# flock-lab/flock

Hardware: AMD Instinct MI355X
Metric: NEXMark rows/sec per node (q3 join, q5 agg) (higher is better)
Workload: dtype int32; 1 GPU; NEXMark q5 hopping(10,5) over 1087 s x 1000000 events/s per GPU; query=q5, input_rows_per_gpu=1000040000, windows_per_gpu=216, parallelism=one GPU, one process

## Files before the change

### flock_amd/csrc/q5.hip

```cpp
#include <algorithm>

#include "sort.hpp"

using namespace flockgpu;

namespace {

constexpr int kQ5Iters = 8;
constexpr int kQ5Tile = kBlock * 4 * kQ5Iters;
constexpr int kHist = 4096;
constexpr int kHistPad = 64;
constexpr int kSlots = kHist / 2;
constexpr int kSlotBits = 11;
static_assert(kSlots == (1 << kSlotBits), "slot bits");
constexpr int kLdsMaxProbe = 24;
constexpr uint32_t kFib = 0x9E3779B1u;
constexpr int kHotMin = 16;
constexpr int kMaxWinPanes = 8;
constexpr uint32_t kWideTile = 0x40000000u;

struct PaneDesc {
    int64_t base;
    uint64_t cnt_off;
    uint32_t range;
    uint32_t pad;
};

struct WinDesc {
    int64_t base;
    uint32_t range;
    int32_t pane_lo, pane_hi;
    uint32_t pad;
};

__device__ __forceinline__ int lds_hash_insert(uint64_t *tab, uint32_t key, uint32_t c) {
    uint32_t s = (key * kFib) >> (32 - kSlotBits);
    const uint64_t mine = ((uint64_t)key << 32) | c;
#pragma unroll 1
    for (int probe = 0; probe < kLdsMaxProbe; ++probe) {
        uint64_t cur = __hip_atomic_load(&tab[s], __ATOMIC_RELAXED, __HIP_MEMORY_SCOPE_WORKGROUP);
        if (cur == 0) {
            cur = atomicCAS(reinterpret_cast<unsigned long long *>(&tab[s]), 0ull, (unsigned long long)mine);
            if (cur == 0) return 2;
        }
        if ((uint32_t)(cur >> 32) == key) {
            atomicAdd(reinterpret_cast<unsigned long long *>(&tab[s]), (unsigned long long)c);
            return 1;
        }
        s = (s + 1) & (kSlots - 1);
    }
    return 0;
}

__device__ __forceinline__ void table_add(uint64_t *tab, uint32_t cap, uint32_t key, uint32_t c, uint32_t *used, uint32_t *err) {
    uint32_t s = (uint32_t)(((uint64_t)(key * kFib) * cap) >> 32);
    const uint64_t mine = ((uint64_t)key << 32) | c;
#pragma unroll 1
    for (uint32_t probe = 0, lim = cap < 2048u ? cap : 2048u; probe < lim; ++probe) {
        uint64_t cur = __hip_atomic_load(&tab[s], __ATOMIC_RELAXED, __HIP_MEMORY_SCOPE_AGENT);
        if (cur == 0) {
            uint64_t expected = 0;
            if (__hip_atomic_compare_exchange_strong(&tab[s], &expected, mine, __ATOMIC_RELAXED, __ATOMIC_RELAXED,
                                                     __HIP_MEMORY_SCOPE_AGENT)) {
                if (*used == 0) *used = 1u;
                return;
            }
            cur = expected;
        }
        if ((uint32_t)(cur >> 32) == key) {
            __hip_atomic_fetch_add(&tab[s], (uint64_t)c, __ATOMIC_RELAXED, __HIP_MEMORY_SCOPE_AGENT);
            return;
        }
        s = (s + 1 == cap) ? 0 : s + 1;
    }
    atomicOr(err, 1u);
}

__device__ __forceinline__ uint32_t table_find(const uint64_t *tab, uint32_t cap, uint32_t key) {
    uint32_t s = (uint32_t)(((uint64_t)(key * kFib) * cap) >> 32);
#pragma unroll 1
    for (uint32_t probe = 0, lim = cap < 2048u ? cap : 2048u; probe < lim; ++probe) {
        const uint64_t cur = tab[s];
        if (cur == 0) return 0;
        if ((uint32_t)(cur >> 32) == key) return (uint32_t)cur;
        s = (s + 1 == cap) ? 0 : s + 1;
    }
    return 0;
}

struct FlushArgs {
    PaneDesc pane;
    int32_t wp0, wp1;
    const int32_t *pane_win_idx;
    uint32_t *counters;
    uint64_t *tables;
    uint32_t cap;
    uint32_t *tab_used;
    uint32_t *err;
    bool c16 = false;
    unsigned long long *tab_rows = nullptr;
};

// ... 78 lines not shown
    uint64_t capacity, budget_bytes;
    PaneDesc *panes;
    WinDesc *wins;
    uint64_t *info;
};
__device__ __forceinline__ void q5_layout_block(const int32_t *__restrict__ rng, const int32_t *__restrict__ pane_win_ptr,
                                                const int64_t *__restrict__ seg_off, int32_t n_panes, int32_t n_win,
                                                uint64_t capacity, uint64_t budget_bytes, PaneDesc *__restrict__ panes,
                                                WinDesc *__restrict__ wins, uint64_t *__restrict__ info) {
    __shared__ uint64_t s_wave[kWavesPerBlock];
    __shared__ uint64_t s_carry;
    __shared__ int s_ok;
    const int lane = lane_id(), wave = threadIdx.x >> 6;
    if (threadIdx.x == 0) {
        s_carry = 0;
        s_ok = 1;
    }
    __syncthreads();
    for (int32_t p0 = 0; p0 < n_panes; p0 += kBlock) {
        const int32_t p = p0 + (int32_t)threadIdx.x;
        int64_t base = 0, range = 0;
        if (p < n_panes && pane_win_ptr[p + 1] != pane_win_ptr[p] && seg_off[2 * p + 1] > seg_off[2 * p]) {
            int32_t mn = 0x7fffffff, mx = (int32_t)0x80000000;
            for (int b = 0; b < kRangeBlocks; ++b) {
                mn = min(mn, rng[((size_t)p * kRangeBlocks + b) * 2]);
                mx = max(mx, rng[((size_t)p * kRangeBlocks + b) * 2 + 1]);
            }
            if (mn <= mx && !q5_pane_layout(mn, mx, &base, &range)) {
                s_ok = 0;
                range = 0;
            }
        }
        const uint64_t incl = wave_incl_scan_u64((uint64_t)range);
        if (lane == 63) s_wave[wave] = incl;
        __syncthreads();
        uint64_t off = s_carry + incl - (uint64_t)range;
        for (int v = 0; v < wave; ++v) off += s_wave[v];
        if (p < n_panes) panes[p] = PaneDesc{base, off, (uint32_t)range, 0};
        __syncthreads();
        if (threadIdx.x == kBlock - 1) s_carry = off + (uint64_t)range;
        __syncthreads();
    }
    const uint64_t cnt_total = s_carry;
    __syncthreads();
    uint64_t scan = 0;
    for (int32_t w = threadIdx.x; w < n_win; w += kBlock) {
        WinDesc d = wins[w];
        int64_t lo = INT64_MAX, hi = INT64_MIN;
        for (int32_t p = d.pane_lo; p < d.pane_hi; ++p) {
            const PaneDesc pd = panes[p];
            if (pd.range) {
                lo = lo < pd.base ? lo : pd.base;
                hi = hi > pd.base + (int64_t)pd.range ? hi : pd.base + (int64_t)pd.range;
            }
        }
        d.base = 0;
        d.range = 0;
        if (lo < hi) {
            if (hi - lo >= (int64_t(1) << 31)) s_ok = 0;
            else {
                d.base = lo;
                d.range = (uint32_t)(hi - lo);
                scan += (uint64_t)(hi - lo);
            }
        }
        wins[w] = d;
    }
    scan = wave_sum_u64(scan);
    if (lane == 0) s_wave[wave] = scan;
    __syncthreads();
    if (threadIdx.x == 0) {
        uint64_t scan_total = 0;
        for (int v = 0; v < kWavesPerBlock; ++v) scan_total += s_wave[v];
        const bool ok = s_ok && cnt_total <= capacity && cnt_total * 4 <= budget_bytes && scan_total * 4 <= 2 * budget_bytes;
        info[0] = cnt_total;
        info[1] = scan_total;
        info[2] = ok ? 1 : 0;
    }
}

__global__ __launch_bounds__(kBlock) void q5_clear_kernel(uint32_t *__restrict__ counters, uint64_t cnt_host,
                                                          uint64_t cnt_from, uint64_t *__restrict__ tables, uint64_t table_words,
                                                          uint64_t *__restrict__ meta, uint64_t meta_words, int32_t *__restrict__ slow_list,
                                                          uint32_t *__restrict__ block_max, uint64_t block_max_words, int c16, LayoutArgs lay) {
    if (lay.rng && blockIdx.x == 0) q5_layout_block(lay.rng, lay.pane_win_ptr, lay.seg_off, lay.n_panes, lay.n_win, lay.capacity, lay.budget_bytes, lay.panes, lay.wins, lay.info);
    uint64_t cnt = cnt_host;
    if (c16) cnt = (cnt + 1) / 2;
    const uint64_t i0 = (uint64_t)blockIdx.x * kBlock + threadIdx.x, stride = (uint64_t)gridDim.x * kBlock;
    const uint4 z = make_uint4(0, 0, 0, 0);
    for (uint64_t i = i0 + cnt_from / 4; i * 4 < cnt + 3; i += stride) {
        uint32_t *p = counters + i * 4;
        __builtin_nontemporal_store(0u, p);
        __builtin_nontemporal_store(0u, p + 1);
        __builtin_nontemporal_store(0u, p + 2);
        __builtin_nontemporal_store(0u, p + 3);
    }
    for (uint64_t i = i0; i * 2 < table_words; i += stride) {
        if (i * 2 + 1 < table_words) reinterpret_cast<uint4 *>(tables)[i] = z;
        else tables[i * 2] = 0;
    }
    for (uint64_t i = i0; i < meta_words; i += stride) meta[i] = 0;
    for (uint64_t i = i0; i < block_max_words; i += stride) block_max[i] = 0;
    if (i0 == 0) slow_list[0] = 0;
}

template <bool kWeighted>
__device__ __forceinline__ void q5_count_tile(const int32_t *__restrict__ auction, const uint32_t *__restrict__ weight, const SegTiles &st,
                                              const PaneDesc *__restrict__ panes, const int32_t *__restrict__ pane_win_ptr,
                                              const int32_t *__restrict__ pane_win_idx, uint32_t *counters, uint64_t *tables, uint32_t cap,
                                              uint32_t *tab_used, uint32_t *err, int32_t *slow_list, unsigned long long *pane_wsum, const int32_t tile,
                                              uint32_t *hist, int32_t *s_red, unsigned long long *s_w, const bool c16, unsigned long long *tab_rows) {
    const TileRange tr = locate_tile(st, tile, kQ5Tile);
    FlushArgs f;
    f.c16 = c16;
    f.tab_rows = tab_rows ? tab_rows + tr.seg : nullptr;
    f.wp0 = pane_win_ptr[tr.seg];
    f.wp1 = pane_win_ptr[tr.seg + 1];
    if (f.wp0 == f.wp1) return;
    f.pane = panes[tr.seg];
    f.pane_win_idx = pane_win_idx;
    f.counters = counters;
    f.tables = tables;
    f.cap = cap;
    f.tab_used = tab_used;
    f.err = err;
    const bool full_tile = tr.lo == tr.tile_begin && tr.hi == tr.tile_begin + kQ5Tile;
    if (kWeighted) {
        unsigned long long wsum = 0;
        constexpr int kChunks = kQ5Tile / kBlock, kBatch = 8;
#pragma unroll 1
        for (int c0 = 0; c0 < kChunks; c0 += kBatch) {
            int32_t kk[kBatch];
            uint32_t ww[kBatch];
#pragma unroll
            for (int b = 0; b < kBatch; ++b) {
                const int64_t r = tr.tile_begin + (int64_t)(c0 + b) * kBlock + threadIdx.x;
                const bool in = full_tile || (r >= tr.lo && r < tr.hi);
                kk[b] = in ? __builtin_nontemporal_load(&auction[r]) : 0;
                ww[b] = in ? __builtin_nontemporal_load(&weight[r]) : 0u;
            }
#pragma unroll
            for (int b = 0; b < kBatch; ++b)
                if (ww[b]) {
                    emit_pair(kk[b], ww[b], f);
                    wsum += ww[b];
                }
        }
        wsum = wave_sum_u64(wsum);
        if (lane_id() == 0) s_w[threadIdx.x >> 6] = wsum;
        __syncthreads();
        if (threadIdx.x == 0 && pane_wsum) {
            const unsigned long long tot = s_w[0] + s_w[1] + s_w[2] + s_w[3];
            if (tot) atomicAdd(&pane_wsum[tr.seg], tot);
        }
        return;
    }
    {
        uint4 *z = reinterpret_cast<uint4 *>(hist);
        for (int s = threadIdx.x; s < (kHist + kHistPad) / 4; s += kBlock) z[s] = make_uint4(0, 0, 0, 0);
    }
    const int lane = lane_id(), wave = threadIdx.x >> 6;
    int32_t k[kQ5Iters][4];
    const int32_t key0 = full_tile ? 0 : auction[tr.lo];
    if (full_tile) {
#pragma unroll
        for (int it = 0; it < kQ5Iters; ++it) {
            const int64_t r0 = tr.tile_begin + it * (kBlock * 4) + threadIdx.x * 4;
            const int4 t = stream_load4(auction + r0);
            k[it][0] = t.x; k[it][1] = t.y; k[it][2] = t.z; k[it][3] = t.w;
// ... 413 lines not shown
        if (lane_id() == 0) {
            s_best[threadIdx.x >> 6] = best;
            s_groups[threadIdx.x >> 6] = g;
        }
        __syncthreads();
        if (threadIdx.x == 0) {
            uint32_t b = 0;
            uint64_t gs = 0;
#pragma unroll
            for (int v = 0; v < kWavesPerBlock; ++v) {
                b = max(b, s_best[v]);
                gs += s_groups[v];
            }
            if (b) block_max[(size_t)w * gridDim.x + blockIdx.x] = b;
            if (b) atomicMax(reinterpret_cast<unsigned long long *>(&win_max[w]), (unsigned long long)b);
            if (gs) atomicAdd(reinterpret_cast<unsigned long long *>(&win_groups[w]), (unsigned long long)gs);
        }
    }
}

template <bool SELECT, bool k16>
__global__ __launch_bounds__(kBlock) void q5_hop2_scan_kernel(const PaneDesc *__restrict__ panes, const int32_t *__restrict__ pane_wa,
                                                              const int32_t *__restrict__ pane_wb, const uint32_t *__restrict__ counters,
                                                              const uint64_t *__restrict__ tables, uint32_t cap, const uint32_t *__restrict__ tab_used,
                                                              uint64_t *win_max, uint64_t *win_groups, uint32_t *block_max, uint32_t *cursor,
                                                              uint32_t out_cap, int32_t *out_win, int32_t *out_key, const uint64_t *__restrict__ spec_info,
                                                              unsigned long long *pane_sum) {
    constexpr int G = k16 ? 8 : 4;
    __shared__ uint32_t s_best[2][kWavesPerBlock];
    __shared__ uint64_t s_groups[3][kWavesPerBlock];
    if (spec_info && !spec_info[2]) return;
    const int32_t p = blockIdx.y;
    const int32_t wa = pane_wa[p], wb = pane_wb[p];
    if (wa < 0 && wb < 0) return;
    const PaneDesc pd = panes[p];
    const PaneDesc prev = wa >= 0 ? panes[p - 1] : PaneDesc{0, 0, 0, 0};
    const bool two_b = wb >= 0 && pane_wa[p + 1] == wb;
    const PaneDesc next = two_b ? panes[p + 1] : PaneDesc{0, 0, 0, 0};
    const uint32_t mx_a = SELECT && wa >= 0 ? (uint32_t)win_max[wa] : 0u, mx_b = SELECT && wb >= 0 ? (uint32_t)win_max[wb] : 0u;
    bool act_a = wa >= 0, act_b = wb >= 0;
    if (SELECT) {
        act_a = act_a && mx_a != 0 && block_max[((size_t)wa * 2 + 1) * gridDim.x + blockIdx.x] == mx_a;
        act_b = act_b && mx_b != 0 && block_max[((size_t)wb * 2 + 0) * gridDim.x + blockIdx.x] == mx_b;
        if (!act_a && !act_b) return;
    }
    const bool tab_a = wa >= 0 && tab_used[wa] != 0, tab_b = wb >= 0 && tab_used[wb] != 0;
    const uint64_t *ta = tables + (size_t)(wa >= 0 ? wa : 0) * cap, *tb = tables + (size_t)(wb >= 0 ? wb : 0) * cap;
    uint32_t best_a = 0, best_b = 0, groups_a = 0, groups_b = 0;
    uint64_t sum = 0;
    auto take = [&](uint32_t c, int32_t key, int32_t w, uint32_t mx, uint32_t &best, uint32_t &groups) {
        if (SELECT) {
            const bool hit = c == mx;
            const uint64_t b = __ballot(hit);
            if (b) {
                const int leader = __ffsll((unsigned long long)b) - 1;
                uint32_t base = 0;
                if (lane_id() == leader) base = atomicAdd(cursor, (uint32_t)__popcll((unsigned long long)b));
                base = __builtin_amdgcn_readlane(base, leader);
                const uint32_t pos = base + mbcnt(b);
                if (hit && pos < out_cap) {
                    out_win[pos] = w;
                    out_key[pos] = key;
                }
            }
        } else {
            best = max(best, c);
            groups += c != 0;
        }
    };
    auto unpack = [&](const uint4 v, uint32_t (&c)[G]) {
        if constexpr (k16) {
            const uint32_t w[4] = {v.x, v.y, v.z, v.w};
#pragma unroll
            for (int j = 0; j < 4; ++j) {
                c[2 * j] = w[j] & 0xFFFFu;
                c[2 * j + 1] = w[j] >> 16;
            }
        } else {
            c[0] = v.x; c[1] = v.y; c[2] = v.z; c[3] = v.w;
        }
    };
    const uint32_t ng = pd.range / G;
    const uint32_t *mine = counters + (k16 ? pd.cnt_off / 2 : pd.cnt_off), *theirs = counters + (k16 ? next.cnt_off / 2 : next.cnt_off);
    for (uint32_t i = blockIdx.x * kBlock + threadIdx.x; i < ng; i += gridDim.x * kBlock) {
        const int64_t k0 = pd.base + (int64_t)i * G;
        uint32_t me[G];
        unpack(*reinterpret_cast<const uint4 *>(mine + (uint64_t)i * 4), me);
        if (k16 && !SELECT) {
#pragma unroll
            for (int j = 0; j < G; ++j) sum += me[j];
        }
        if (act_b) {
            uint32_t c[G];
#pragma unroll
            for (int j = 0; j < G; ++j) c[j] = me[j];
            const uint64_t idx = (uint64_t)(k0 - next.base);
            if (idx < (uint64_t)next.range) {
                uint32_t o[G];
                unpack(*reinterpret_cast<const uint4 *>(theirs + (k16 ? idx / 2 : idx)), o);
#pragma unroll
                for (int j = 0; j < G; ++j) c[j] += o[j];
            }
            if (tab_b) {
#pragma unroll
                for (int j = 0; j < G; ++j) c[j] += table_find(tb, cap, (uint32_t)(int32_t)(k0 + j));
            }
#pragma unroll
            for (int j = 0; j < G; ++j) take(c[j], (int32_t)(k0 + j), wb, mx_b, best_b, groups_b);
        }
        if (act_a && !((uint64_t)(k0 - prev.base) < (uint64_t)prev.range)) {
            uint32_t c[G];
#pragma unroll
            for (int j = 0; j < G; ++j) c[j] = me[j];
            if (tab_a) {
#pragma unroll
                for (int j = 0; j < G; ++j) c[j] += table_find(ta, cap, (uint32_t)(int32_t)(k0 + j));
            }
#pragma unroll
            for (int j = 0; j < G; ++j) take(c[j], (int32_t)(k0 + j), wa, mx_a, best_a, groups_a);
        }
    }
    if (tab_b && act_b) {
        for (uint32_t sl = blockIdx.x * kBlock + threadIdx.x; sl < cap; sl += gridDim.x * kBlock) {
            const uint64_t e = tb[sl];
            if (!e) continue;
            const int64_t key = (int32_t)(uint32_t)(e >> 32);
            if ((uint64_t)(key - pd.base) < (uint64_t)pd.range || (uint64_t)(key - next.base) < (uint64_t)next.range) continue;
            if (SELECT) {
                if ((uint32_t)e == mx_b) {
                    const uint32_t pos = atomicAdd(cursor, 1u);
                    if (pos < out_cap) {
                        out_win[pos] = wb;
                        out_key[pos] = (int32_t)key;
                    }
                }
            } else {
                best_b = max(best_b, (uint32_t)e);
                groups_b += 1;
            }
        }
    }
    if (!SELECT) {
        const uint32_t ba = wave_max_u32(best_a), bb = wave_max_u32(best_b);
        const uint64_t ga = wave_sum_u64(groups_a), gb = wave_sum_u64(groups_b), gs = k16 ? wave_sum_u64(sum) : 0;
        if (lane_id() == 0) {
            s_best[0][threadIdx.x >> 6] = ba;
            s_best[1][threadIdx.x >> 6] = bb;
            s_groups[0][threadIdx.x >> 6] = ga;
            s_groups[1][threadIdx.x >> 6] = gb;
            s_groups[2][threadIdx.x >> 6] = gs;
        }
        __syncthreads();
        if (threadIdx.x < 2) {
            const int r = threadIdx.x;
            const int32_t w = r == 0 ? wa : wb;
            uint32_t b = 0;
            uint64_t g = 0;
#pragma unroll
            for (int v = 0; v < kWavesPerBlock; ++v) {
                b = max(b, s_best[r][v]);
                g += s_groups[r][v];
            }
            if (w >= 0) {
                if (b) block_max[((size_t)w * 2 + (r == 0 ? 1 : 0)) * gridDim.x + blockIdx.x] = b;
                if (b) atomicMax(reinterpret_cast<unsigned long long *>(&win_max[w]), (unsigned long long)b);
                if (g) atomicAdd(reinterpret_cast<unsigned long long *>(&win_groups[w]), (unsigned long long)g);
// ... 494 lines not shown
    if (preclean.size() != 2) preclean.assign(2, 0);
    LayoutArgs lay{};
    uint64_t clean_upto = 0;
    const bool c16 = !weight && !part && !wide_mode && hop2 && ctx->host_i64["q5.no_c16"].empty();
    auto words_of = [&](uint64_t n_counters) -> uint64_t { return c16 ? (n_counters + 1) / 2 : n_counters; };
    if (speculate) {
        FG_TRY(arena_get_t(ctx, "q5.counters", (size_t)words_of((uint64_t)hint[0] + (uint64_t)hint[0] / 8) + 8, &counters));
        capacity = (ctx->arena["q5.counters"].cap / sizeof(uint32_t) - 8) * (c16 ? 2 : 1);
        if (preclean[0] == (int64_t)reinterpret_cast<uintptr_t>(counters)) clean_upto = (uint64_t)preclean[1];
        {
            std::vector<int64_t> &wsig = ctx->host_i64["q5.wins_sig"];
            std::vector<int64_t> wnow;
            wnow.reserve((size_t)2 * n_win + 2);
            wnow.push_back((int64_t)reinterpret_cast<uintptr_t>(d_wins));
            for (int w = 0; w < n_win; ++w) {
                wnow.push_back(win->win_pane_lo[w]);
                wnow.push_back(win->win_pane_hi[w]);
            }
            if (wsig != wnow) {
                std::copy(wins.begin(), wins.end(), h_wins);
                FG_HIP(ctx, hipMemcpyAsync(d_wins, h_wins, wins.size() * sizeof(WinDesc), hipMemcpyHostToDevice, ctx->stream));
                wsig = wnow;
            }
        }
        lay = LayoutArgs{d_rng, d_ptr, st.seg_off, n_panes, n_win, capacity, budget, d_panes, d_wins, d_info};
        cnt_total = (uint64_t)hint[0];
        scan_total = (uint64_t)hint[1];
    } else {
        FG_TRY(upload_layout());
        FG_TRY(arena_get_t(ctx, "q5.counters", (size_t)words_of(cnt_total) + 8, &counters));
    }
    preclean[0] = preclean[1] = 0;

    const size_t n_meta = (size_t)2 * n_win + 1 + ((size_t)n_win + 1) / 2 + 1;
    const size_t n_meta_all = n_meta + (size_t)2 * std::max(n_panes, 0);
    uint64_t *d_meta = nullptr, *h_meta = nullptr;
    FG_TRY(arena_get_t(ctx, "q5.meta", n_meta_all, &d_meta));
    unsigned long long *d_pane_sum = reinterpret_cast<unsigned long long *>(d_meta + n_meta), *d_tab_rows = d_pane_sum + std::max(n_panes, 0);
    FG_TRY(pinned_get_t(ctx, "q5.meta", n_meta, &h_meta));
    uint32_t *d_cursor = reinterpret_cast<uint32_t *>(d_meta + 2 * n_win), *d_err = d_cursor + 1, *d_used = d_cursor + 2;

    unsigned long long *d_wsum = nullptr, *h_wsum = nullptr;
    if (weight && n_panes > 0) {
        FG_TRY(arena_get_t(ctx, "q5.pane_weight", (size_t)n_panes + 1, &d_wsum));
        FG_TRY(pinned_get_t(ctx, "q5.pane_weight", (size_t)n_panes + 1, &h_wsum));
    }
    double rpg = ctx->q5_rows_per_group < 1.0 ? 1.0 : ctx->q5_rows_per_group;
    uint64_t cap64 = dense ? 1024 : std::max<uint64_t>(1024, (uint64_t)((double)max_win_rows / rpg * 2.0) + 64);
    uint32_t out_cap = 1u << 16;
    std::vector<int32_t> h_win, h_key;
    uint32_t n_sel = 0;
    const int32_t *sel_win = nullptr, *sel_key = nullptr;
    bool fin_sorted = false;
    const int64_t *fin_off = nullptr;
    const int32_t *fin_auction = nullptr;
    const uint64_t *fin_num = nullptr;
    uint32_t h_slow_count = 0;
    for (int attempt = 0;; ++attempt) {
        if (attempt > 8 || cap64 >= (uint64_t(1) << 31))
            return fail(ctx, FLOCKGPU_ERR_CAPACITY, "q5: hash table capacity %llu still overflows", (unsigned long long)cap64);
        const uint32_t cap = (uint32_t)cap64;
        const uint64_t *spec_info = speculate ? d_info : nullptr;
        uint64_t *tables = nullptr;
        FG_TRY(arena_get_t(ctx, "q5.tables", (size_t)cap * std::max(n_win, 1), &tables));
        int32_t *o_win = nullptr, *o_key = nullptr, *slow_list = nullptr;
        FG_TRY(arena_get_t(ctx, "q5.sel_win", out_cap, &o_win));
        FG_TRY(arena_get_t(ctx, "q5.sel_key", out_cap, &o_key));
        FG_TRY(arena_get_t(ctx, "q5.slow_list", (size_t)st.n_tiles + 2, &slow_list));
        const uint64_t per_win = n_win > 0 ? std::max<uint64_t>(cap, scan_total / n_win / 4) : cap;
        const bool pane_walk = hop2;
        const uint64_t per_pane = n_panes > 0 ? std::max<uint64_t>(cap, cnt_total / (uint64_t)n_panes / 4) : cap;
        const int hop2_blocks = c16 ? 16 : 32;
        const unsigned gx = (unsigned)std::min<int64_t>(std::max<int64_t>(div_up((int64_t)(pane_walk ? per_pane : per_win), kBlock * 2), 1), pane_walk ? hop2_blocks : 64);
        uint32_t *block_max = nullptr;
        const uint64_t n_block_max = (uint64_t)gx * std::max(n_win, 1) * (pane_walk ? 2 : 1);
        FG_TRY(arena_get_t(ctx, "q5.block_max", (size_t)n_block_max, &block_max));
        {
            const uint64_t clear_words = std::max<uint64_t>({words_of(speculate ? capacity : cnt_total), (uint64_t)cap * n_win, (uint64_t)n_meta_all, n_block_max});
            const unsigned cg = (unsigned)std::max<int64_t>(1, std::min<int64_t>(div_up((int64_t)clear_words / 4 + 1, kBlock), (int64_t)ctx->num_cus * 16));
            {
                LaunchScope ls(ctx, "q5_clear_kernel");
                hipLaunchKernelGGL(q5_clear_kernel, dim3(cg), dim3(kBlock), 0, ctx->stream, counters, speculate ? capacity : cnt_total,
                                   (attempt == 0 && speculate) ? (clean_upto & ~uint64_t(3)) : uint64_t(0), tables, (uint64_t)cap * n_win, d_meta, (uint64_t)n_meta_all,
                                   slow_list, block_max, n_block_max, c16 ? 1 : 0, speculate ? lay : LayoutArgs{});
                if (speculate) clean_upto = std::max(clean_upto, words_of(capacity));
            }
            FG_TRY(check_launch(ctx, "q5_clear_kernel"));
        }
        if (d_wsum) FG_HIP(ctx, hipMemsetAsync(d_wsum, 0, sizeof(unsigned long long) * (size_t)n_panes, ctx->stream));
        uint32_t nd = 0;
        if (wide_mode && dense) {
            uint32_t max_range = 0;
            for (int p = 0; p < n_panes; ++p) max_range = std::max(max_range, panes[(size_t)p].range);
            nd = (uint32_t)div_up((int64_t)max_range, int64_t(1) << kPartShift) + 1;
        }
        const bool wide = wide_mode && dense && nd >= 2 && nd <= (uint32_t)kPartMaxDigits && st.n_tiles > 0 && n_win > 0;
        wide_ran = wide;
        uint32_t *d_sample = nullptr, *h_sample = nullptr;
        FG_TRY(arena_get_t(ctx, "q5.part_sample", 4, &d_sample));
        FG_TRY(pinned_get_t(ctx, "q5.part_sample", 4, &h_sample));
        h_sample[0] = h_sample[1] = 0;
        if (wide) {
            SegTiles st4;
            FG_TRY(build_seg_tiles(ctx, "q5.part", sb.data(), se.data(), n_panes, kPartTile, &st4));
            const int64_t slots = (int64_t)st4.n_tiles * (nd + 1);
            if (slots >= (int64_t(1) << 31)) return fail(ctx, FLOCKGPU_ERR_UNSUPPORTED, "q5: too many (pane, digit, tile) slots for the partition pass");
            int32_t *off_mat = nullptr, *part_keys = nullptr;
            uint16_t *part_low = nullptr;
            FG_TRY(arena_get_t(ctx, "q5.part_hist", (size_t)slots + 4, &off_mat));
            FG_TRY(arena_get_t(ctx, "q5.part_keys", (size_t)st4.n_tiles * kPartTile + 4, &part_keys));
            FG_TRY(arena_get_t(ctx, "q5.part_low", (size_t)st4.n_tiles * kPartTile + 8, &part_low));
            FG_HIP(ctx, hipMemsetAsync(d_sample, 0, 2 * sizeof(uint32_t), ctx->stream));
            {
                LaunchScope ls(ctx, "q5_part_tile_kernel");
                hipLaunchKernelGGL(q5_part_tile_kernel, dim3((unsigned)st4.n_tiles), dim3(kBlock), 0, ctx->stream, auction, st4, d_panes, d_ptr, nd, off_mat, part_keys,
                                   part_low, d_sample);
            }
            FG_TRY(check_launch(ctx, "q5_part_tile_kernel"));
            {
                LaunchScope ls(ctx, "q5_bucket_count_kernel");
                hipLaunchKernelGGL(q5_bucket_count_kernel, dim3(nd, (unsigned)n_panes), dim3(kBlock), 0, ctx->stream, part_keys, part_low, st4, d_panes, d_ptr, d_idx, nd,
                                   off_mat, counters, tables, cap, d_used, d_err);
            }
            FG_TRY(check_launch(ctx, "q5_bucket_count_kernel"));
            FG_HIP(ctx, hipMemcpyAsync(h_sample, d_sample, 2 * sizeof(uint32_t), hipMemcpyDeviceToHost, ctx->stream));
        } else if (st.n_tiles > 0 && n_win > 0) {
            {
                LaunchScope ls(ctx, "q5_count_kernel");
                hipLaunchKernelGGL(weight ? q5_count_kernel<true> : q5_count_kernel<false>, dim3((unsigned)st.n_tiles), dim3(kBlock), 0,
                                   ctx->stream, auction, weight, st, d_panes, d_ptr, d_idx, counters, tables, cap, d_used, d_err,
                                   slow_list, spec_info, d_wsum, c16 ? 1 : 0, c16 ? d_tab_rows : (unsigned long long *)nullptr);
            }
            FG_TRY(check_launch(ctx, "q5_count_kernel"));
            if (d_wsum) FG_HIP(ctx, hipMemcpyAsync(h_wsum, d_wsum, sizeof(unsigned long long) * (size_t)n_panes, hipMemcpyDeviceToHost, ctx->stream));
            {
                LaunchScope ls(ctx, "q5_count_slow_kernel");
                const unsigned gs = (unsigned)std::min<int64_t>(st.n_tiles, (int64_t)ctx->num_cus * 8);
                hipLaunchKernelGGL(weight ? q5_count_slow_kernel<true> : q5_count_slow_kernel<false>, dim3(gs), dim3(kBlock), 0,
                                   ctx->stream, auction, weight, st, d_panes, d_ptr, d_idx, counters, tables, cap, d_used, d_err,
                                   slow_list, spec_info, c16 ? 1 : 0, c16 ? d_tab_rows : (unsigned long long *)nullptr);
            }
            FG_TRY(check_launch(ctx, "q5_count_slow_kernel"));
        }
        if (part) {
            const int64_t tab0 = ((int64_t)cnt_total + 3) & ~int64_t(3);
            std::vector<int64_t> xb((size_t)2 * n_win), xe((size_t)2 * n_win);
            for (int w = 0; w < n_win; ++w) {
                xb[2 * w] = (int64_t)panes[w].cnt_off;
                xe[2 * w] = (int64_t)panes[w].cnt_off + (int64_t)panes[w].range;
                xb[2 * w + 1] = tab0 + (int64_t)w * cap;
                xe[2 * w + 1] = xb[2 * w + 1] + cap;
            }
            SegTiles sx;
            FG_TRY(build_seg_tiles(ctx, "q5.partial", xb.data(), xe.data(), 2 * n_win, kFlagTile, &sx));
            uint32_t *x_flags = nullptr, *x_counts = nullptr;
            uint64_t *x_base = nullptr;
            int64_t *d_xoff = nullptr, *h_xoff = nullptr;
            FG_TRY(arena_get_t(ctx, "q5.partial_flags", (size_t)sx.n_tiles * kBlock + 4, &x_flags));
            FG_TRY(arena_get_t(ctx, "q5.partial_counts", (size_t)sx.n_tiles * kWavesPerBlock + 4, &x_counts));
            FG_TRY(arena_get_t(ctx, "q5.partial_base", (size_t)sx.n_tiles + 1, &x_base));
            FG_TRY(arena_get_t(ctx, "q5.partial_off", (size_t)2 * n_win + 1, &d_xoff));
            FG_TRY(pinned_get_t(ctx, "q5.partial_off", (size_t)2 * n_win + 1, &h_xoff));
            if (sx.n_tiles > 0) {
                LaunchScope ls(ctx, "q5_partial_flag_kernel");
                hipLaunchKernelGGL(q5_partial_flag_kernel, dim3((unsigned)sx.n_tiles), dim3(kBlock), 0, ctx->stream, sx, counters, tables,
                                   tab0, x_flags, x_counts);
            }
            FG_TRY(check_launch(ctx, "q5_partial_flag_kernel"));
            FG_TRY(launch_tile_scan(ctx, x_counts, sx.n_tiles, x_base, sx.tile_first, sx.n_seg, d_xoff));
            FG_HIP(ctx, hipMemcpyAsync(h_xoff, d_xoff, sizeof(int64_t) * ((size_t)2 * n_win + 1), hipMemcpyDeviceToHost, ctx->stream));
            FG_HIP(ctx, hipMemcpyAsync(h_meta, d_meta, sizeof(uint64_t) * n_meta, hipMemcpyDeviceToHost, ctx->stream));
            FG_HIP(ctx, hipStreamSynchronize(ctx->stream));
            if (reinterpret_cast<const uint32_t *>(h_meta + 2 * n_win)[1]) {
                cap64 *= 4;
                continue;
            }
            const int64_t n_out = h_xoff[2 * n_win];
            if (n_out >= (int64_t(1) << 31)) return fail(ctx, FLOCKGPU_ERR_UNSUPPORTED, "q5 partial: more than 2^31 groups");
            int32_t *p_key = nullptr;
            uint32_t *p_cnt = nullptr;
            FG_TRY(arena_get_t(ctx, "q5.partial_key", (size_t)n_out + 4, &p_key));
            FG_TRY(arena_get_t(ctx, "q5.partial_cnt", (size_t)n_out + 4, &p_cnt));
            if (sx.n_tiles > 0 && n_out > 0) {
                LaunchScope ls(ctx, "q5_partial_emit_kernel");
                hipLaunchKernelGGL(q5_partial_emit_kernel, dim3((unsigned)sx.n_tiles), dim3(kBlock), 0, ctx->stream, sx, x_flags, x_counts,
                                   x_base, counters, tables, tab0, d_panes, p_key, p_cnt);
            }
            FG_TRY(check_launch(ctx, "q5_partial_emit_kernel"));
            std::vector<int64_t> &poffs = ctx->host_i64["q5.partial_pane_offsets"];
            poffs.resize((size_t)n_win + 1);
            for (int w = 0; w <= n_win; ++w) poffs[w] = h_xoff[2 * w];
            part->auction = p_key;
            part->count = p_cnt;
            part->pane_out_offsets = poffs.data();
            part->rows = n_out;
            return FLOCKGPU_OK;
        }
        if (n_win > 0 && pane_walk) {
            {
                LaunchScope ls(ctx, "q5_max_kernel");
                hipLaunchKernelGGL((c16 ? q5_hop2_scan_kernel<false, true> : q5_hop2_scan_kernel<false, false>), dim3(gx, (unsigned)n_panes), dim3(kBlock), 0, ctx->stream, d_panes, d_roles,
                                   d_roles + role_a.size(), counters, tables, cap, d_used, d_meta, d_meta + n_win, block_max, d_cursor, out_cap, o_win, o_key, spec_info, d_pane_sum);
            }
            FG_TRY(check_launch(ctx, "q5_max_kernel"));
            {
                LaunchScope ls(ctx, "q5_select_kernel");
                hipLaunchKernelGGL((c16 ? q5_hop2_scan_kernel<true, true> : q5_hop2_scan_kernel<true, false>), dim3(gx, (unsigned)n_panes), dim3(kBlock), 0, ctx->stream, d_panes, d_roles,
                                   d_roles + role_a.size(), counters, tables, cap, d_used, d_meta, d_meta + n_win, block_max, d_cursor, out_cap, o_win, o_key, spec_info, d_pane_sum);
            }
            FG_TRY(check_launch(ctx, "q5_select_kernel"));
        } else if (n_win > 0) {
            {
                LaunchScope ls(ctx, "q5_max_kernel");
                hipLaunchKernelGGL(q5_scan_kernel<false>, dim3(gx, (unsigned)n_win), dim3(kBlock), 0, ctx->stream, d_wins,
                                   d_panes, counters, tables, cap, d_used, d_meta, d_meta + n_win, block_max, d_cursor, out_cap,
                                   o_win, o_key, spec_info);
            }
            FG_TRY(check_launch(ctx, "q5_max_kernel"));
            {
                LaunchScope ls(ctx, "q5_select_kernel");
                hipLaunchKernelGGL(q5_scan_kernel<true>, dim3(gx, (unsigned)n_win), dim3(kBlock), 0, ctx->stream, d_wins,
                                   d_panes, counters, tables, cap, d_used, d_meta, d_meta + n_win, block_max, d_cursor, out_cap,
                                   o_win, o_key, spec_info);
            }
            FG_TRY(check_launch(ctx, "q5_select_kernel"));
        }
        constexpr uint32_t kSpecWinners = 4096;
        uint64_t *h_fin = nullptr;
        int32_t *fin_a = nullptr;
        uint64_t *fin_n = nullptr;
        FG_TRY(pinned_get_t(ctx, "q5.finish", n_meta + 8 + (size_t)n_win + 2, &h_fin));
        FG_TRY(arena_get_t(ctx, "q5.out_auction", (size_t)kFinishMax + 1, &fin_a));
        FG_TRY(arena_get_t(ctx, "q5.out_num", (size_t)kFinishMax + 1, &fin_n));
        {
            LaunchScope ls(ctx, "q5_finish_kernel");
            hipLaunchKernelGGL(q5_finish_kernel, dim3(1), dim3(kFinishThreads), 0, ctx->stream, d_meta, (uint32_t)n_meta, n_win, spec_info, slow_list, o_win, o_key, out_cap,
                               fin_a, fin_n, h_fin, c16 && pane_walk ? d_pane_sum : (const unsigned long long *)nullptr, d_tab_rows, st.seg_off, d_ptr, n_panes);
        }
        FG_TRY(check_launch(ctx, "q5_finish_kernel"));
        FG_HIP(ctx, hipStreamSynchronize(ctx->stream));
        std::copy(h_fin, h_fin + n_meta, h_meta);
        if (speculate) std::copy(h_fin + n_meta, h_fin + n_meta + 3, h_info);
        h_slow_count = (uint32_t)h_fin[n_meta + 3];
        if (h_fin[n_meta + 3] >> 32) {
            ctx->host_i64["q5.no_c16"].assign(1, 1);
            return q5_run(ctx, auction, weight, rows, win, out, part);
        }
        fin_sorted = h_fin[n_meta + 4] != 0;
        fin_off = reinterpret_cast<const int64_t *>(h_fin + n_meta + 5);
        if (speculate) {
            if (!h_info[2]) {
                speculate = false;
                hint[2] = 0;
                FG_TRY(host_layout());
                FG_TRY(upload_layout());
                FG_TRY(arena_get_t(ctx, "q5.counters", (size_t)words_of(cnt_total) + 8, &counters));
                cap64 = dense ? 1024 : std::max<uint64_t>(1024, (uint64_t)((double)max_win_rows / rpg * 2.0) + 64);
                --attempt;
                continue;
            }
            cnt_total = h_info[0];
            scan_total = h_info[1];
        }
        if (h_wsum) {
            for (int w = 0; w < n_win; ++w) {
                unsigned long long tot = 0;
                for (int p = win->win_pane_lo[w]; p < win->win_pane_hi[w]; ++p) tot += h_wsum[p];
                if (tot >= (1ull << 32))
                    return fail(ctx, FLOCKGPU_ERR_UNSUPPORTED, "q5 weighted: the counts of window %d add up to %llu >= 2^32 (32-bit counters)", w, tot);
            }
        }
        const uint32_t *tail = reinterpret_cast<const uint32_t *>(h_meta + 2 * n_win);
        n_sel = tail[0];
        if (tail[1]) {
            cap64 *= 4;
            continue;
        }
        if (n_sel > out_cap) {
            out_cap = n_sel + 1024;
            continue;
        }
        h_win.resize(n_sel);
        h_key.resize(n_sel);
        if (fin_sorted) {
            fin_auction = fin_a;
            fin_num = fin_n;
        } else if (n_sel <= kSpecWinners) {
            FG_HIP(ctx, hipMemcpyAsync(h_win.data(), o_win, sizeof(int32_t) * n_sel, hipMemcpyDeviceToHost, ctx->stream));
            FG_HIP(ctx, hipMemcpyAsync(h_key.data(), o_key, sizeof(int32_t) * n_sel, hipMemcpyDeviceToHost, ctx->stream));
            FG_HIP(ctx, hipStreamSynchronize(ctx->stream));
        } else {
            sel_win = o_win;
            sel_key = o_key;
        }
        break;
    }
    hint[0] = (int64_t)cnt_total;
    hint[1] = (int64_t)scan_total;
    hint[2] = dense ? 1 : 0;
    if (!weight && !part) {
        uint32_t *h_sample = nullptr;
        FG_TRY(pinned_get_t(ctx, "q5.part_sample", 4, &h_sample));
        if (wide_mode && !wide_ran) wide_hint[0] = 0;
        else if (wide_mode && h_sample[0]) wide_hint[0] = (uint64_t)h_sample[1] * 4 >= (uint64_t)h_sample[0] * 3 ? 0 : 1;
        else if (!wide_mode && dense && st.n_tiles > 64) wide_hint[0] = (int64_t)h_slow_count * 4 > (int64_t)st.n_tiles ? 1 : 0;
    }
    {
        double best = 1e30;
        for (int w = 0; w < n_win; ++w) {
            const int64_t rows = win->pane_row_offsets[win->win_pane_hi[w]] - win->pane_row_offsets[win->win_pane_lo[w]];
            const uint64_t g = h_meta[n_win + w];
            if (g) best = std::min(best, (double)rows / (double)g);
        }
        if (best < 1e30) ctx->q5_rows_per_group = best;
    }
    std::vector<int64_t> &offs = ctx->host_i64["q5.win_out_offsets"];
    std::vector<uint64_t> &wmax = ctx->host_u64["q5.win_max"], &wgrp = ctx->host_u64["q5.win_groups"];
    offs.assign((size_t)n_win + 1, 0);
    wmax.assign(h_meta, h_meta + n_win);
    wgrp.assign(h_meta + n_win, h_meta + 2 * n_win);
    if (fin_sorted) {
        offs.assign(fin_off, fin_off + n_win + 1);
        out->auction = fin_auction;
        out->num = fin_num;
        out->win_out_offsets = offs.data();
        out->win_max = wmax.data();
        out->win_groups = wgrp.data();
        out->rows = n_sel;
    } else
    if (sel_key) {
        int32_t *d_mm = nullptr, *h_mm = nullptr, *k1 = nullptr, *w_in = nullptr, *w2 = nullptr, *d_oa = nullptr;
        uint32_t *v1 = nullptr, *v2 = nullptr;
        uint64_t *d_on = nullptr;
        int64_t *d_off = nullptr, *h_off = nullptr;
        FG_TRY(arena_get_t(ctx, "q5.ord_minmax", 4, &d_mm));
        FG_TRY(pinned_get_t(ctx, "q5.ord_minmax", 4, &h_mm));
        FG_TRY(key_min_max(ctx, sel_key, n_sel, d_mm));
        FG_HIP(ctx, hipMemcpyAsync(h_mm, d_mm, 2 * sizeof(int32_t), hipMemcpyDeviceToHost, ctx->stream));
        FG_HIP(ctx, hipStreamSynchronize(ctx->stream));
        int bits = 1, wbits = 1;
        while (bits < 32 && (((uint64_t)((int64_t)h_mm[1] - (int64_t)h_mm[0])) >> bits)) ++bits;
        while (wbits < 31 && ((uint32_t)n_win >> wbits)) ++wbits;
        FG_TRY(radix_sort_pairs(ctx, "q5.ord_key", sel_key, nullptr, n_sel, h_mm[0], bits, &k1, &v1));
        FG_TRY(arena_get_t(ctx, "q5.ord_win_in", (size_t)n_sel + 4, &w_in));
        FG_TRY(gather_i32(ctx, sel_win, reinterpret_cast<const int32_t *>(v1), n_sel, w_in));
        FG_TRY(radix_sort_pairs(ctx, "q5.ord_win", w_in, v1, n_sel, 0, wbits, &w2, &v2));
        FG_TRY(arena_get_t(ctx, "q5.out_auction", (size_t)n_sel + 1, &d_oa));
        FG_TRY(arena_get_t(ctx, "q5.out_num", (size_t)n_sel + 1, &d_on));
        FG_TRY(arena_get_t(ctx, "q5.ord_off", (size_t)n_win + 2, &d_off));
        FG_TRY(pinned_get_t(ctx, "q5.ord_off", (size_t)n_win + 2, &h_off));
        FG_TRY(gather_i32(ctx, sel_key, reinterpret_cast<const int32_t *>(v2), n_sel, d_oa));
        hipLaunchKernelGGL(q5_winner_num_kernel, dim3((unsigned)div_up((int64_t)n_sel, kBlock)), dim3(kBlock), 0, ctx->stream, w2,
                           d_meta, (int64_t)n_sel, d_on);
        FG_TRY(check_launch(ctx, "q5_winner_num_kernel"));
        FG_TRY(sorted_key_offsets(ctx, w2, n_sel, n_win, d_off));
        FG_HIP(ctx, hipMemcpyAsync(h_off, d_off, sizeof(int64_t) * ((size_t)n_win + 1), hipMemcpyDeviceToHost, ctx->stream));
        FG_HIP(ctx, hipStreamSynchronize(ctx->stream));
        offs.assign(h_off, h_off + n_win + 1);
        out->auction = d_oa;
        out->num = d_on;
        out->win_out_offsets = offs.data();
        out->win_max = wmax.data();
        out->win_groups = wgrp.data();
        out->rows = n_sel;
        return FLOCKGPU_OK;
    }
    if (!fin_sorted) {
    std::vector<uint32_t> order(n_sel);
    for (uint32_t i = 0; i < n_sel; ++i) order[i] = i;
    std::sort(order.begin(), order.end(), [&](uint32_t a, uint32_t b) {
        return h_win[a] != h_win[b] ? h_win[a] < h_win[b] : h_key[a] < h_key[b];
    });
    int32_t *h_oa = nullptr;
    uint64_t *h_on = nullptr;
    FG_TRY(pinned_get_t(ctx, "q5.out_auction", (size_t)n_sel + 1, &h_oa));
    FG_TRY(pinned_get_t(ctx, "q5.out_num", (size_t)n_sel + 1, &h_on));
    for (uint32_t i = 0; i < n_sel; ++i) {
        const uint32_t s = order[i];
        h_oa[i] = h_key[s];
        h_on[i] = wmax[h_win[s]];
        offs[h_win[s] + 1] += 1;
    }
    for (int w = 0; w < n_win; ++w) offs[w + 1] += offs[w];
    int32_t *d_oa = nullptr;
    uint64_t *d_on = nullptr;
    FG_TRY(arena_get_t(ctx, "q5.out_auction", (size_t)n_sel + 1, &d_oa));
    FG_TRY(arena_get_t(ctx, "q5.out_num", (size_t)n_sel + 1, &d_on));
    if (n_sel) {
        FG_HIP(ctx, hipMemcpyAsync(d_oa, h_oa, sizeof(int32_t) * n_sel, hipMemcpyHostToDevice, ctx->stream));
        FG_HIP(ctx, hipMemcpyAsync(d_on, h_on, sizeof(uint64_t) * n_sel, hipMemcpyHostToDevice, ctx->stream));
    }
    out->auction = d_oa;
    out->num = d_on;
    out->win_out_offsets = offs.data();
    out->win_max = wmax.data();
    out->win_groups = wgrp.data();
    out->rows = n_sel;
    }
    if (speculate && dense && cnt_total > 0) {
        int32_t *slow_list = nullptr;
        FG_TRY(arena_get_t(ctx, "q5.slow_list", (size_t)st.n_tiles + 2, &slow_list));
        {
            LaunchScope ls(ctx, "q5_clear_kernel");
            const unsigned cg = (unsigned)std::max<int64_t>(1, std::min<int64_t>(div_up((int64_t)words_of(cnt_total) / 4 + 1, kBlock), (int64_t)ctx->num_cus * 16));
            hipLaunchKernelGGL(q5_clear_kernel, dim3(cg), dim3(kBlock), 0, ctx->stream, counters, cnt_total, uint64_t(0), (uint64_t *)nullptr,
                               uint64_t(0), (uint64_t *)nullptr, uint64_t(0), slow_list, (uint32_t *)nullptr, uint64_t(0), c16 ? 1 : 0, LayoutArgs{});
        }
        FG_TRY(check_launch(ctx, "q5_clear_kernel"));
        preclean[0] = (int64_t)reinterpret_cast<uintptr_t>(counters);
        preclean[1] = (int64_t)std::max<uint64_t>(clean_upto, words_of(cnt_total));
    }
    return FLOCKGPU_OK;
}

namespace flockgpu {

int q5_partial_by_tile(flockgpu_ctx *ctx, const flockgpu_bid_cols *bid, const flockgpu_windows *win, Q5TilePartial *out) {
    *out = Q5TilePartial{};
    FG_TRY(check_windows(ctx, win, bid->rows, "q5 partial"));
    if (bid->rows > 0 && !bid->auction) return fail(ctx, FLOCKGPU_ERR_INVALID, "q5 partial: null auction column");
    if (reinterpret_cast<uintptr_t>(bid->auction) & 15) return fail(ctx, FLOCKGPU_ERR_UNSUPPORTED, "q5: auction column must be 16-byte aligned");
    if (bid->rows >= (int64_t(1) << 31)) return fail(ctx, FLOCKGPU_ERR_UNSUPPORTED, "q5 partial: more than 2^31 rows per call");
    FG_HIP(ctx, hipSetDevice(ctx->device));
    const int n_panes = win->n_panes;
    std::vector<char> used((size_t)std::max(n_panes, 1), 0);
    for (int w = 0; w < win->n_windows; ++w)
        for (int p = win->win_pane_lo[w]; p < win->win_pane_hi[w]; ++p) used[(size_t)p] = 1;
    std::vector<int64_t> sb((size_t)n_panes), se((size_t)n_panes);
    for (int p = 0; p < n_panes; ++p) {
        sb[(size_t)p] = win->pane_row_offsets[p];
        se[(size_t)p] = win->pane_row_offsets[p + 1];
    }
    SegTiles st;
    FG_TRY(build_seg_tiles(ctx, "q5.tile_panes", sb.data(), se.data(), n_panes, kQ5Tile, &st));
    int64_t *d_reg = nullptr, *h_reg = nullptr;
    uint32_t *d_cur = nullptr, *h_cur = nullptr;
    int32_t *o_key = nullptr;
    uint32_t *o_cnt = nullptr;
    FG_TRY(arena_get_t(ctx, "q5.tile_region", (size_t)n_panes + 1, &d_reg));
    FG_TRY(pinned_get_t(ctx, "q5.tile_region", (size_t)n_panes + 1, &h_reg));
    FG_TRY(arena_get_t(ctx, "q5.tile_cursor", (size_t)n_panes + 1, &d_cur));
    FG_TRY(pinned_get_t(ctx, "q5.tile_cursor", (size_t)n_panes + 1, &h_cur));
    FG_TRY(arena_get_t(ctx, "q5.tile_key", (size_t)bid->rows + 4, &o_key));
    FG_TRY(arena_get_t(ctx, "q5.tile_cnt", (size_t)bid->rows + 4, &o_cnt));
    for (int p = 0; p < n_panes; ++p) h_reg[p] = used[(size_t)p] ? sb[(size_t)p] : -1;
    FG_HIP(ctx, hipMemcpyAsync(d_reg, h_reg, sizeof(int64_t) * (size_t)std::max(n_panes, 1), hipMemcpyHostToDevice, ctx->stream));
    FG_HIP(ctx, hipMemsetAsync(d_cur, 0, sizeof(uint32_t) * ((size_t)n_panes + 1), ctx->stream));
    int64_t max_tiles = 0;
    for (int p = 0; p < n_panes; ++p)
        if (se[(size_t)p] > sb[(size_t)p]) max_tiles = std::max(max_tiles, div_up(se[(size_t)p] - (sb[(size_t)p] & ~int64_t(3)), (int64_t)kQ5Tile));
    if (max_tiles * n_panes >= (int64_t(1) << 31)) return fail(ctx, FLOCKGPU_ERR_UNSUPPORTED, "q5 partial: too many (pane, tile) pairs");
    if (st.n_tiles > 0) {
        LaunchScope ls(ctx, "q5_partial_tile_kernel");
        hipLaunchKernelGGL(q5_partial_tile_kernel, dim3((unsigned)(max_tiles * n_panes)), dim3(kBlock), 0, ctx->stream, bid->auction, st, d_reg, d_cur, o_key,
                           o_cnt);
    }
    FG_TRY(check_launch(ctx, "q5_partial_tile_kernel"));
    FG_HIP(ctx, hipMemcpyAsync(h_cur, d_cur, sizeof(uint32_t) * (size_t)std::max(n_panes, 1), hipMemcpyDeviceToHost, ctx->stream));
    FG_HIP(ctx, hipStreamSynchronize(ctx->stream));
    out->auction = o_key;
    out->count = o_cnt;
    out->capacity = bid->rows;
    out->offsets.resize((size_t)2 * n_panes + 1);
    for (int p = 0; p < n_panes; ++p) {
        const int64_t n = used[(size_t)p] ? (int64_t)h_cur[p] : 0;
        if (n > se[(size_t)p] - sb[(size_t)p]) return fail(ctx, FLOCKGPU_ERR_HIP, "q5 partial: pane %d claims %lld pairs for %lld rows", p, (long long)n, (long long)(se[(size_t)p] - sb[(size_t)p]));
        out->offsets[(size_t)2 * p] = sb[(size_t)p];
        out->offsets[(size_t)2 * p + 1] = sb[(size_t)p] + n;
        out->pairs += n;
    }
    out->offsets[(size_t)2 * n_panes] = n_panes ? se[(size_t)n_panes - 1] : 0;
    return FLOCKGPU_OK;
}

}

extern "C" {

int flockgpu_q5_hot_items(flockgpu_ctx *ctx, const flockgpu_bid_cols *bid, const flockgpu_windows *win,
                          flockgpu_q5_result *out) {
    if (!ctx) return FLOCKGPU_ERR_INVALID;
    if (!bid || !out || bid->rows < 0) return fail(ctx, FLOCKGPU_ERR_INVALID, "q5: null argument");
    return q5_run(ctx, bid->auction, nullptr, bid->rows, win, out, nullptr);
}

int flockgpu_q5_hot_items_weighted(flockgpu_ctx *ctx, const int32_t *auction, const uint32_t *count, int64_t rows,
                                   const flockgpu_windows *win, flockgpu_q5_result *out) {
    if (!ctx) return FLOCKGPU_ERR_INVALID;
    if (!out || rows < 0 || (rows > 0 && (!auction || !count))) return fail(ctx, FLOCKGPU_ERR_INVALID, "q5 weighted: null argument");
    return q5_run(ctx, auction, count, rows, win, out, nullptr);
}
// ... 17 lines not shown
```

Measured before the change: 1312 billion rows/s.

## Pack 16-bit counter scan and overlap counter clear with finish readback

```diff
diff --git a/flock_amd/csrc/q5.hip b/flock_amd/csrc/q5.hip
--- a/flock_amd/csrc/q5.hip
+++ b/flock_amd/csrc/q5.hip
@@ -18,6 +18,14 @@
 constexpr int kHotMin = 16;
 constexpr int kMaxWinPanes = 8;
 constexpr uint32_t kWideTile = 0x40000000u;
+
+using u16x2 = unsigned short __attribute__((ext_vector_type(2)));
+__device__ __forceinline__ u16x2 as_u16x2(uint32_t w) { return __builtin_bit_cast(u16x2, w); }
+__device__ __forceinline__ u16x2 nonzero_u16x2(u16x2 c) {
+    uint32_t r;
+    asm("v_pk_min_u16 %0, %1, %2" : "=v"(r) : "v"(__builtin_bit_cast(uint32_t, c)), "s"(0x00010001u));
+    return as_u16x2(r);
+}
 
 struct PaneDesc {
     int64_t base;
@@ -262,9 +270,11 @@
 __global__ __launch_bounds__(kBlock) void q5_clear_kernel(uint32_t *__restrict__ counters, uint64_t cnt_host,
                                                           uint64_t cnt_from, uint64_t *__restrict__ tables, uint64_t table_words,
                                                           uint64_t *__restrict__ meta, uint64_t meta_words, int32_t *__restrict__ slow_list,
-                                                          uint32_t *__restrict__ block_max, uint64_t block_max_words, int c16, LayoutArgs lay) {
+                                                          uint32_t *__restrict__ block_max, uint64_t block_max_words, int c16, LayoutArgs lay,
+                                                          const uint64_t *__restrict__ cnt_info) {
     if (lay.rng && blockIdx.x == 0) q5_layout_block(lay.rng, lay.pane_win_ptr, lay.seg_off, lay.n_panes, lay.n_win, lay.capacity, lay.budget_bytes, lay.panes, lay.wins, lay.info);
     uint64_t cnt = cnt_host;
+    if (cnt_info) cnt = cnt_info[2] ? (cnt_info[0] < cnt_host ? cnt_info[0] : cnt_host) : 0;
     if (c16) cnt = (cnt + 1) / 2;
     const uint64_t i0 = (uint64_t)blockIdx.x * kBlock + threadIdx.x, stride = (uint64_t)gridDim.x * kBlock;
     const uint4 z = make_uint4(0, 0, 0, 0);
@@ -844,6 +854,61 @@
     };
     const uint32_t ng = pd.range / G;
     const uint32_t *mine = counters + (k16 ? pd.cnt_off / 2 : pd.cnt_off), *theirs = counters + (k16 ? next.cnt_off / 2 : next.cnt_off);
+    bool packed_done = false;
+    if constexpr (k16 && !SELECT) {
+        if (!tab_a && !tab_b) {
+            packed_done = true;
+            const u16x2 one = {1, 1};
+            u16x2 pk_a = {0, 0}, pk_b = {0, 0};
+            uint32_t sum32 = 0;
+            const uint32_t i_first = blockIdx.x * kBlock + threadIdx.x, i_step = gridDim.x * kBlock;
+            for (uint32_t i = i_first; i < ng; i += i_step) {
+                const int64_t k0 = pd.base + (int64_t)i * G;
+                const uint64_t idx = (uint64_t)(k0 - next.base);
+                const bool cov = act_b && idx < (uint64_t)next.range;
+                const uint4 m4 = *reinterpret_cast<const uint4 *>(mine + (uint64_t)i * 4);
+                uint4 o4 = *reinterpret_cast<const uint4 *>(theirs + (cov ? idx / 2 : uint64_t(0)));
+                o4.x = cov ? o4.x : 0u;
+                o4.y = cov ? o4.y : 0u;
+                o4.z = cov ? o4.z : 0u;
+                o4.w = cov ? o4.w : 0u;
+                const uint32_t mw[4] = {m4.x, m4.y, m4.z, m4.w}, ow[4] = {o4.x, o4.y, o4.z, o4.w};
+#pragma unroll
+                for (int j = 0; j < 4; ++j) sum32 = __builtin_amdgcn_udot2(as_u16x2(mw[j]), one, sum32, false);
+                if (act_b) {
+#pragma unroll
+                    for (int j = 0; j < 4; ++j) {
+                        const u16x2 c = __builtin_elementwise_add_sat(as_u16x2(mw[j]), as_u16x2(ow[j]));
+                        pk_b = __builtin_elementwise_max(pk_b, c);
+                        groups_b = __builtin_amdgcn_udot2(nonzero_u16x2(c), one, groups_b, false);
+                    }
+                }
+                if (act_a && !((uint64_t)(k0 - prev.base) < (uint64_t)prev.range)) {
+#pragma unroll
+                    for (int j = 0; j < 4; ++j) {
+                        const u16x2 c = as_u16x2(mw[j]);
+                        pk_a = __builtin_elementwise_max(pk_a, c);
+                        groups_a = __builtin_amdgcn_udot2(nonzero_u16x2(c), one, groups_a, false);
+                    }
+                }
+            }
+            sum = sum32;
+            best_a = max((uint32_t)pk_a.x, (uint32_t)pk_a.y);
+            best_b = max((uint32_t)pk_b.x, (uint32_t)pk_b.y);
+            if (best_b == 0xFFFFu) {
+                for (uint32_t i = i_first; i < ng; i += i_step) {
+                    const uint64_t idx = (uint64_t)(pd.base + (int64_t)i * G - next.base);
+                    if (!(idx < (uint64_t)next.range)) continue;
+                    uint32_t me[G], o[G];
+                    unpack(*reinterpret_cast<const uint4 *>(mine + (uint64_t)i * 4), me);
+                    unpack(*reinterpret_cast<const uint4 *>(theirs + idx / 2), o);
+#pragma unroll
+                    for (int j = 0; j < G; ++j) best_b = max(best_b, me[j] + o[j]);
+                }
+            }
+        }
+    }
+    if (!packed_done)
     for (uint32_t i = blockIdx.x * kBlock + threadIdx.x; i < ng; i += gridDim.x * kBlock) {
         const int64_t k0 = pd.base + (int64_t)i * G;
         uint32_t me[G];
@@ -1504,7 +1569,7 @@
                 LaunchScope ls(ctx, "q5_clear_kernel");
                 hipLaunchKernelGGL(q5_clear_kernel, dim3(cg), dim3(kBlock), 0, ctx->stream, counters, speculate ? capacity : cnt_total,
                                    (attempt == 0 && speculate) ? (clean_upto & ~uint64_t(3)) : uint64_t(0), tables, (uint64_t)cap * n_win, d_meta, (uint64_t)n_meta_all,
-                                   slow_list, block_max, n_block_max, c16 ? 1 : 0, speculate ? lay : LayoutArgs{});
+                                   slow_list, block_max, n_block_max, c16 ? 1 : 0, speculate ? lay : LayoutArgs{}, (const uint64_t *)nullptr);
                 if (speculate) clean_upto = std::max(clean_upto, words_of(capacity));
             }
             FG_TRY(check_launch(ctx, "q5_clear_kernel"));
@@ -1654,13 +1719,26 @@
         FG_TRY(pinned_get_t(ctx, "q5.finish", n_meta + 8 + (size_t)n_win + 2, &h_fin));
         FG_TRY(arena_get_t(ctx, "q5.out_auction", (size_t)kFinishMax + 1, &fin_a));
         FG_TRY(arena_get_t(ctx, "q5.out_num", (size_t)kFinishMax + 1, &fin_n));
+        const bool poll = !d_wsum && !wide;
+        if (poll) pinned_pending(h_fin, (int)(n_meta + 5 + (size_t)n_win + 1));
         {
             LaunchScope ls(ctx, "q5_finish_kernel");
             hipLaunchKernelGGL(q5_finish_kernel, dim3(1), dim3(kFinishThreads), 0, ctx->stream, d_meta, (uint32_t)n_meta, n_win, spec_info, slow_list, o_win, o_key, out_cap,
                                fin_a, fin_n, h_fin, c16 && pane_walk ? d_pane_sum : (const unsigned long long *)nullptr, d_tab_rows, st.seg_off, d_ptr, n_panes);
         }
         FG_TRY(check_launch(ctx, "q5_finish_kernel"));
-        FG_HIP(ctx, hipStreamSynchronize(ctx->stream));
+        if (speculate && dense) {
+            LaunchScope ls(ctx, "q5_clear_kernel");
+            const unsigned cg = (unsigned)std::max<int64_t>(1, std::min<int64_t>(div_up((int64_t)words_of(cnt_total) / 4 + 1, kBlock), (int64_t)ctx->num_cus * 16));
+            hipLaunchKernelGGL(q5_clear_kernel, dim3(cg), dim3(kBlock), 0, ctx->stream, counters, capacity, uint64_t(0), (uint64_t *)nullptr,
+                               uint64_t(0), (uint64_t *)nullptr, uint64_t(0), slow_list, (uint32_t *)nullptr, uint64_t(0), c16 ? 1 : 0, LayoutArgs{}, d_info);
+        }
+        FG_TRY(check_launch(ctx, "q5_clear_kernel"));
+        if (poll) {
+            FG_TRY(wait_pinned(ctx, h_fin, (int)(n_meta + 5)));
+            if (h_fin[n_meta + 4]) FG_TRY(wait_pinned(ctx, h_fin + n_meta + 5, n_win + 1));
+        } else
+            FG_HIP(ctx, hipStreamSynchronize(ctx->stream));
         std::copy(h_fin, h_fin + n_meta, h_meta);
         if (speculate) std::copy(h_fin + n_meta, h_fin + n_meta + 3, h_info);
         h_slow_count = (uint32_t)h_fin[n_meta + 3];
@@ -1820,15 +1898,6 @@
     out->rows = n_sel;
     }
     if (speculate && dense && cnt_total > 0) {
-        int32_t *slow_list = nullptr;
-        FG_TRY(arena_get_t(ctx, "q5.slow_list", (size_t)st.n_tiles + 2, &slow_list));
-        {
-            LaunchScope ls(ctx, "q5_clear_kernel");
-            const unsigned cg = (unsigned)std::max<int64_t>(1, std::min<int64_t>(div_up((int64_t)words_of(cnt_total) / 4 + 1, kBlock), (int64_t)ctx->num_cus * 16));
-            hipLaunchKernelGGL(q5_clear_kernel, dim3(cg), dim3(kBlock), 0, ctx->stream, counters, cnt_total, uint64_t(0), (uint64_t *)nullptr,
-                               uint64_t(0), (uint64_t *)nullptr, uint64_t(0), slow_list, (uint32_t *)nullptr, uint64_t(0), c16 ? 1 : 0, LayoutArgs{});
-        }
-        FG_TRY(check_launch(ctx, "q5_clear_kernel"));
         preclean[0] = (int64_t)reinterpret_cast<uintptr_t>(counters);
         preclean[1] = (int64_t)std::max<uint64_t>(clean_upto, words_of(cnt_total));
     }
```

Measured after the change: 1343 billion rows/s, median of 6. +2.4%, better.
